# christhetree/mod_extraction

Hardware: AMD Instinct MI355X
Metric: 44.1 kHz audio-seconds/sec (train step), interwoven ph/fl/ch (higher is better)
Workload: dtype f32

## Files before the change

### mod_extraction_amd/csrc/wgrad_kvec_f16.hip

```cpp
#include "conv_common.h"
#include <stdlib.h>

typedef _Float16 half8 __attribute__((ext_vector_type(8)));
typedef _Float16 half4 __attribute__((ext_vector_type(4)));
typedef short short4v __attribute__((__vector_size__(4 * sizeof(short))));

#define WK_KS_MAX 6
#define WK_CH (WK_KS_MAX * 32)
#define WK_AP (WK_CH + 16)
#define WK_BR (WK_CH + 12)

#define WK_A_BYTES (2 * 64 * WK_AP * 2)
#define WK_B_ROWS ((WK_BR + 7) / 8 * 8)
#define WK_LDS_BYTES (WK_A_BYTES + 2 * WK_B_ROWS * 32)

struct WgradKvecArgs {
    const float *G;
    const unsigned char *amax;
    const float *scale;
    const _Float16 *xk_hi, *xk_lo;
    float *part;
    int B, H, Wv, rows_per_slab, n_slabs;
    int packed;
};

__device__ __forceinline__ floatx4 mfma_16x16x32(half8 a, half8 b, floatx4 c)
{
    return __builtin_amdgcn_mfma_f32_16x16x32_f16(a, b, c, 0, 0, 0);
}

__device__ __forceinline__ int wk_a_slot(int c8) { return c8 < 4 ? 8 * c8 : 8 * (c8 - 4) + 4; }
__device__ __forceinline__ half8 tr_frag16(const unsigned char *img, int lane_off, int r0)
{
    const unsigned char *ptr = img + lane_off + r0 * 32;
    const short4v v0 = __builtin_amdgcn_ds_read_tr16_b64_v4i16((short4v __attribute__((address_space(3))) *)ptr);
    const short4v v1 = __builtin_amdgcn_ds_read_tr16_b64_v4i16((short4v __attribute__((address_space(3))) *)(ptr + 16 * 32));
    typedef short short8v __attribute__((__vector_size__(8 * sizeof(short))));
    const short8v both = __builtin_shufflevector(v0, v1, 0, 1, 2, 3, 4, 5, 6, 7);
    return __builtin_bit_cast(half8, both);
}

__global__ __launch_bounds__(256, 2) void wgrad_kvec_f16_kernel(WgradKvecArgs a)
{
    extern __shared__ __attribute__((aligned(256))) unsigned char wk_smem[];
    _Float16 *const dzA = reinterpret_cast<_Float16 *>(wk_smem);
    _Float16 *const xB = reinterpret_cast<_Float16 *>(wk_smem + WK_A_BYTES);
    const int tid = threadIdx.x, lane = tid & 63, wave = __builtin_amdgcn_readfirstlane(tid >> 6);
    const int tap0 = wave * 3 + (wave >> 1);
    const int m16 = lane & 15, kg = lane >> 4;
    const int slab = blockIdx.x;
    const int Hp = a.H >> 1;
    const float S = a.scale[0];

    floatx4 acc[CV_KW];
#pragma unroll
    for (int i = 0; i < CV_KW; ++i) acc[i] = floatx4{0.f, 0.f, 0.f, 0.f};

    const int a_lane = (m16 * WK_AP + 8 * kg) * 2;
    const int b_lane = (4 * kg + (m16 >> 2)) * 32 + (m16 & 3) * 8;
    constexpr int A_SPLIT = 64 * WK_AP * 2, B_SPLIT = WK_B_ROWS * 32;
    const unsigned char *Ab = reinterpret_cast<const unsigned char *>(dzA);
    const unsigned char *Bb = reinterpret_cast<const unsigned char *>(xB);

    const int row_begin = slab * a.rows_per_slab;
    int row_end = row_begin + a.rows_per_slab;
    if (row_end > a.B * a.H) row_end = a.B * a.H;
    constexpr int NA = 64 * (WK_CH / 4) / 256, NB = (2 * WK_BR * 2 + 255) / 256;
    floatx4 ga[NA], vb[NB];
    unsigned ama[NA];
    auto issue_g = [&](int rid, int w0) {
        const int b = rid / a.H, h = rid - b * a.H;
        const int npos = (CV_PITCH - w0 >= WK_CH) ? WK_CH : (CV_PITCH - w0);
#pragma unroll
        for (int q = 0; q < NA; ++q) {
            const int i = tid + q * 256, co = i / (WK_CH / 4), c4 = i - co * (WK_CH / 4);
            ga[q] = floatx4{0.f, 0.f, 0.f, 0.f};
            ama[q] = 0x02020202u;
            if (c4 * 4 < npos) {
                const size_t off = (((size_t)b * 64 + co) * Hp + (h >> 1)) * CV_PITCH + w0 + c4 * 4;
                ga[q] = __builtin_nontemporal_load(reinterpret_cast<const floatx4 *>(a.G + off));
                ama[q] = __builtin_nontemporal_load(reinterpret_cast<const unsigned *>(a.amax + off));
            }
        }
    };
    auto issue_x = [&](int rid, int w0) {
        const int b = rid / a.H, h = rid - b * a.H;
        const int npos = (CV_PITCH - w0 >= WK_CH) ? WK_CH : (CV_PITCH - w0);
#pragma unroll
        for (int q = 0; q < NB; ++q) {
            const int i = tid + q * 256;
            const int split = i / (WK_BR * 2), k = i - split * (WK_BR * 2);
            const int pos = k >> 1, part = k & 1, w = w0 - 6 + pos;
            vb[q] = floatx4{0.f, 0.f, 0.f, 0.f};
            if (i < 2 * WK_BR * 2 && pos < npos + 12 && w >= 0 && w < CV_PITCH)
                vb[q] = *reinterpret_cast<const floatx4 *>((split ? a.xk_lo : a.xk_hi) +
                                                           (((size_t)b * a.H + h) * CV_PITCH + w) * 16 + part * 8);
        }
    };
    auto commit = [&](int rid, int w0) {
        const int h = rid % a.H;
        const unsigned want = (unsigned)(h & 1);
#pragma unroll
        for (int q = 0; q < NA; ++q) {
            const int i = tid + q * 256, co = i / (WK_CH / 4), c4 = i - co * (WK_CH / 4);
            const int wq = w0 + c4 * 4;
            half4 hi, lo;
            if (a.packed) {
                unsigned v[4];
#pragma unroll
                for (int e = 0; e < 4; ++e) v[e] = ((ama[q] >> (8 * e)) & 0xffu) == want ? __float_as_uint(ga[q][e]) : 0u;
                const unsigned h01 = __builtin_amdgcn_perm(v[1], v[0], 0x05040100u), h23 = __builtin_amdgcn_perm(v[3], v[2], 0x05040100u);
                const unsigned l01 = __builtin_amdgcn_perm(v[1], v[0], 0x07060302u), l23 = __builtin_amdgcn_perm(v[3], v[2], 0x07060302u);
                typedef unsigned uintx2 __attribute__((ext_vector_type(2)));
                hi = __builtin_bit_cast(half4, uintx2{h01, h23});
                lo = __builtin_bit_cast(half4, uintx2{l01, l23});
            } else {
#pragma unroll
            for (int e = 0; e < 4; ++e) {
                const bool keep = ((ama[q] >> (8 * e)) & 0xffu) == want && wq + e < a.Wv;
                const float v = keep ? ga[q][e] * S : 0.0f;
                const _Float16 hh = (_Float16)v;
                hi[e] = hh;
                lo[e] = (_Float16)(v - (float)hh);
            }
            }
            const int slot = (c4 >> 3) * 32 + wk_a_slot(c4 & 7);
            *reinterpret_cast<half4 *>(dzA + co * WK_AP + slot) = hi;
            *reinterpret_cast<half4 *>(dzA + 64 * WK_AP + co * WK_AP + slot) = lo;
        }
#pragma unroll
        for (int q = 0; q < NB; ++q) {
            const int i = tid + q * 256;
            if (i < 2 * WK_BR * 2) {
                const int split = i / (WK_BR * 2), k = i - split * (WK_BR * 2);
                *reinterpret_cast<floatx4 *>(xB + (size_t)split * (WK_B_ROWS * 16) + (k >> 1) * 16 + (k & 1) * 8) = vb[q];
            }
        }
    };

    int rid = row_begin, w0 = 0;
    if (rid < row_end) { issue_g(rid, w0); issue_x(rid, w0); }
    while (rid < row_end) {
        const int nks = (CV_PITCH - w0 >= WK_CH) ? WK_KS_MAX : (CV_PITCH - w0) / 32;
        int nrid, nw0 = w0;
        if (!(rid & 1)) nrid = rid + 1;
        else {
            nrid = rid - 1;
            nw0 = w0 + WK_CH;
            if (nw0 >= CV_PITCH) { nw0 = 0; nrid = rid + 1; }
        }
        __syncthreads();
        commit(rid, w0);
        if (nrid < row_end) {
            if (!(nrid & 1)) issue_g(nrid, nw0);
            issue_x(nrid, nw0);
        }
        __syncthreads();
        {
            {
#pragma unroll 1
            for (int ks = 0; ks < nks; ++ks) {
                half8 ah[5], al[5], bh[4], bl[4];
#pragma unroll
                for (int j = 0; j < 5; ++j) {
                    const int jt = j < 4 ? j : wave;
                    ah[j] = *reinterpret_cast<const half8 *>(Ab + a_lane + jt * (16 * WK_AP * 2) + ks * 64);
                    al[j] = *reinterpret_cast<const half8 *>(Ab + A_SPLIT + a_lane + jt * (16 * WK_AP * 2) + ks * 64);
                }
#pragma unroll
                for (int t = 0; t < 4; ++t) {
                    const int kw = t < 3 ? tap0 + t : 6;
                    bh[t] = tr_frag16(Bb, b_lane, ks * 32 + kw);
                    bl[t] = tr_frag16(Bb + B_SPLIT, b_lane, ks * 32 + kw);
                }
#pragma unroll
                for (int u = 0; u < 13; ++u) acc[u] = mfma_16x16x32(al[u < 12 ? (u & 3) : 4], bh[u < 12 ? (u >> 2) : 3], acc[u]);
#pragma unroll
                for (int u = 0; u < 13; ++u) acc[u] = mfma_16x16x32(ah[u < 12 ? (u & 3) : 4], bl[u < 12 ? (u >> 2) : 3], acc[u]);
#pragma unroll
                for (int u = 0; u < 13; ++u) acc[u] = mfma_16x16x32(ah[u < 12 ? (u & 3) : 4], bh[u < 12 ? (u >> 2) : 3], acc[u]);
            }
            }
        }
        rid = nrid;
        w0 = nw0;
    }
#pragma unroll
    for (int u = 0; u < CV_KW; ++u) {
        const int kw = u < 12 ? tap0 + (u >> 2) : 6, j = u < 12 ? (u & 3) : wave;
        float *dst = a.part + (((size_t)slab * CV_KW + kw) * 64 + j * 16) * 16;
#pragma unroll
        for (int r = 0; r < 4; ++r) dst[(4 * kg + r) * 16 + m16] = acc[u][r];
    }
}


__global__ __launch_bounds__(256) void wgrad_kvec_reduce_kernel(const float *__restrict__ part, int n_slabs,
                                                                const float *__restrict__ scale, float *__restrict__ dW)
{
    __shared__ double sh[16][17];
    const int total = CV_KW * 64 * 16;
    const int ol = threadIdx.x & 15, sl = threadIdx.x >> 4;
    const int j = blockIdx.x * 16 + ol;
    double s = 0.0;
    for (int i = sl; i < n_slabs; i += 16) s += (double)part[(size_t)i * total + j];
    sh[sl][ol] = s;
    __syncthreads();
    if (sl == 0) {
        double t = 0.0;
#pragma unroll
        for (int q = 0; q < 16; ++q) t += sh[q][ol];
        const int k = j & 15, co = (j >> 4) & 63, kw = j >> 10;
        if (k < 2 * CV_KH) {
            const int kh = k >> 1, ci = k & 1;
            dW[(((size_t)co * 2 + ci) * CV_KH + kh) * CV_KW + kw] = (float)(t * (double)scale[1]);
        }
    }
}

__global__ void wk_pow2_scale_kernel(const unsigned *__restrict__ amax_bits, float *__restrict__ scale)
{
    const float m = __uint_as_float(*amax_bits);
    int e = 0;
    if (m > 0.0f && m < 3.0e38f) {
        frexpf(m, &e);
        e = 10 - e;
        e = e > 100 ? 100 : (e < -100 ? -100 : e);
    }
    scale[0] = ldexpf(1.0f, e);
    scale[1] = ldexpf(1.0f, -e);
}

MX_EXPORT int mx_conv_block1_wgrad_f16(const float *G, const uint8_t *amax, const uint32_t *amax_bits, const void *xk_hi,
                                       const void *xk_lo, int64_t B, int64_t H, int64_t Wv, int64_t rows_per_slab,
                                       float *scale, float *part, float *dW, void *stream)
{
    if (!G || !amax || !amax_bits || !xk_hi || !xk_lo || !scale || !part || !dW || B <= 0 || rows_per_slab <= 0)
        return MX_ERR_ARG;
    if (H < 2 || (H & 1) || Wv <= 0 || Wv > CV_PITCH) return MX_ERR_UNSUPPORTED;
    rows_per_slab += rows_per_slab & 1;
    const int64_t n_slabs = (B * H + rows_per_slab - 1) / rows_per_slab;
    if (n_slabs > 1000000) return MX_ERR_UNSUPPORTED;
    hipStream_t st = (hipStream_t)stream;
    hipLaunchKernelGGL(wk_pow2_scale_kernel, dim3(1), dim3(1), 0, st, amax_bits, scale);
    WgradKvecArgs a{G, amax, scale, (const _Float16 *)xk_hi, (const _Float16 *)xk_lo, part, (int)B, (int)H, (int)Wv,
                    (int)rows_per_slab, (int)n_slabs, 0};
    static MxLdsLatch latch = {};
    if (mx_set_dyn_lds(latch, (const void *)wgrad_kvec_f16_kernel, WK_LDS_BYTES) != MX_OK) return MX_ERR_LAUNCH;
    hipLaunchKernelGGL(wgrad_kvec_f16_kernel, dim3((unsigned)n_slabs), dim3(256), WK_LDS_BYTES, st, a);
    const int total = CV_KW * 64 * 16;
    hipLaunchKernelGGL(wgrad_kvec_reduce_kernel, dim3(total / 16), dim3(256), 0, st, part, (int)n_slabs, scale, dW);
    return mx_launch_status();
}

MX_EXPORT int mx_conv_block1_wgrad_pair_f16(const void *Gp, const uint8_t *amax, const float *scale, const void *xk_hi,
                                            const void *xk_lo, int64_t B, int64_t H, int64_t Wv, int64_t rows_per_slab,
                                            float *part, float *dW, void *stream)
{
    if (!Gp || !amax || !scale || !xk_hi || !xk_lo || !part || !dW || B <= 0 || rows_per_slab <= 0) return MX_ERR_ARG;
    if (H < 2 || (H & 1) || Wv <= 0 || Wv > CV_PITCH) return MX_ERR_UNSUPPORTED;
    rows_per_slab += rows_per_slab & 1;
    const int64_t n_slabs = (B * H + rows_per_slab - 1) / rows_per_slab;
    if (n_slabs > 1000000) return MX_ERR_UNSUPPORTED;
    hipStream_t st = (hipStream_t)stream;
    WgradKvecArgs a{(const float *)Gp, amax, scale, (const _Float16 *)xk_hi, (const _Float16 *)xk_lo, part, (int)B, (int)H, (int)Wv,
                    (int)rows_per_slab, (int)n_slabs, 1};
    static MxLdsLatch latch = {};
    if (mx_set_dyn_lds(latch, (const void *)wgrad_kvec_f16_kernel, WK_LDS_BYTES) != MX_OK) return MX_ERR_LAUNCH;
    hipLaunchKernelGGL(wgrad_kvec_f16_kernel, dim3((unsigned)n_slabs), dim3(256), WK_LDS_BYTES, st, a);
    const int total = CV_KW * 64 * 16;
    hipLaunchKernelGGL(wgrad_kvec_reduce_kernel, dim3(total / 16), dim3(256), 0, st, part, (int)n_slabs, scale, dW);
    return mx_launch_status();
}
```

Baseline: 7730.

## Use 2:4 sparse SMFMAC for maxpool-masked wgrad, processing row pairs together

The weight-gradient kernel exploits the fact that the maxpool-backward gradient is nonzero in only one row of each H pair. It packs the row pair into a 2:4 structured-sparse A operand with per-lane index bytes and calls smfmac 16x16x64 instead of dense mfma 16x16x32. That halves the MFMA work and lets G/amax be loaded once per pair. The width chunk shrinks from 6 to 4 k-steps, and the LDS layout is reworked to hold interleaved x rows plus a sparsity index buffer. This adds extra index-packing ALU work and more complex transposed LDS reads.

```diff
diff --git a/mod_extraction_amd/csrc/wgrad_kvec_f16.hip b/mod_extraction_amd/csrc/wgrad_kvec_f16.hip
--- a/mod_extraction_amd/csrc/wgrad_kvec_f16.hip
+++ b/mod_extraction_amd/csrc/wgrad_kvec_f16.hip
@@ -1,18 +1,21 @@
 #include "conv_common.h"
 #include <stdlib.h>
 
+typedef _Float16 half16 __attribute__((ext_vector_type(16)));
 typedef _Float16 half8 __attribute__((ext_vector_type(8)));
 typedef _Float16 half4 __attribute__((ext_vector_type(4)));
 typedef short short4v __attribute__((__vector_size__(4 * sizeof(short))));
-
-#define WK_KS_MAX 6
+typedef unsigned uintx2 __attribute__((ext_vector_type(2)));
+
+#define WK_KS_MAX 4
 #define WK_CH (WK_KS_MAX * 32)
 #define WK_AP (WK_CH + 16)
 #define WK_BR (WK_CH + 12)
 
 #define WK_A_BYTES (2 * 64 * WK_AP * 2)
-#define WK_B_ROWS ((WK_BR + 7) / 8 * 8)
-#define WK_LDS_BYTES (WK_A_BYTES + 2 * WK_B_ROWS * 32)
+#define WK_B_SPLIT (WK_BR * 64)
+#define WK_I_BYTES (WK_KS_MAX * 512)
+#define WK_LDS_BYTES (WK_A_BYTES + 2 * WK_B_SPLIT + WK_I_BYTES)
 
 struct WgradKvecArgs {
     const float *G;
@@ -24,27 +27,32 @@
     int packed;
 };
 
-__device__ __forceinline__ floatx4 mfma_16x16x32(half8 a, half8 b, floatx4 c)
-{
-    return __builtin_amdgcn_mfma_f32_16x16x32_f16(a, b, c, 0, 0, 0);
-}
-
-__device__ __forceinline__ int wk_a_slot(int c8) { return c8 < 4 ? 8 * c8 : 8 * (c8 - 4) + 4; }
-__device__ __forceinline__ half8 tr_frag16(const unsigned char *img, int lane_off, int r0)
-{
-    const unsigned char *ptr = img + lane_off + r0 * 32;
-    const short4v v0 = __builtin_amdgcn_ds_read_tr16_b64_v4i16((short4v __attribute__((address_space(3))) *)ptr);
-    const short4v v1 = __builtin_amdgcn_ds_read_tr16_b64_v4i16((short4v __attribute__((address_space(3))) *)(ptr + 16 * 32));
+__device__ __forceinline__ floatx4 smfmac_16x16x64(half8 a, half16 b, floatx4 c, int idx)
+{
+    return __builtin_amdgcn_smfmac_f32_16x16x64_f16(a, b, c, idx, 0, 0);
+}
+
+__device__ __forceinline__ half16 tr_frag64(const unsigned char *img, int off_e, int off_o, int r0)
+{
+    typedef short4v __attribute__((address_space(3))) *lds_p;
+    const short4v v0 = __builtin_amdgcn_ds_read_tr16_b64_v4i16((lds_p)(img + off_e + r0));
+    const short4v v1 = __builtin_amdgcn_ds_read_tr16_b64_v4i16((lds_p)(img + off_o + r0));
+    const short4v v2 = __builtin_amdgcn_ds_read_tr16_b64_v4i16((lds_p)(img + off_e + r0 + 1024));
+    const short4v v3 = __builtin_amdgcn_ds_read_tr16_b64_v4i16((lds_p)(img + off_o + r0 + 1024));
     typedef short short8v __attribute__((__vector_size__(8 * sizeof(short))));
-    const short8v both = __builtin_shufflevector(v0, v1, 0, 1, 2, 3, 4, 5, 6, 7);
-    return __builtin_bit_cast(half8, both);
-}
-
-__global__ __launch_bounds__(256, 2) void wgrad_kvec_f16_kernel(WgradKvecArgs a)
+    typedef short short16v __attribute__((__vector_size__(16 * sizeof(short))));
+    const short8v lo = __builtin_shufflevector(v0, v1, 0, 1, 2, 3, 4, 5, 6, 7);
+    const short8v hi = __builtin_shufflevector(v2, v3, 0, 1, 2, 3, 4, 5, 6, 7);
+    const short16v all = __builtin_shufflevector(lo, hi, 0, 1, 2, 3, 4, 5, 6, 7, 8, 9, 10, 11, 12, 13, 14, 15);
+    return __builtin_bit_cast(half16, all);
+}
+
+__global__ __launch_bounds__(256, 2) void wgrad_kvec_sp_f16_kernel(WgradKvecArgs a)
 {
     extern __shared__ __attribute__((aligned(256))) unsigned char wk_smem[];
     _Float16 *const dzA = reinterpret_cast<_Float16 *>(wk_smem);
-    _Float16 *const xB = reinterpret_cast<_Float16 *>(wk_smem + WK_A_BYTES);
+    unsigned char *const Bb = wk_smem + WK_A_BYTES;
+    unsigned char *const Ib = wk_smem + WK_A_BYTES + 2 * WK_B_SPLIT;
     const int tid = threadIdx.x, lane = tid & 63, wave = __builtin_amdgcn_readfirstlane(tid >> 6);
     const int tap0 = wave * 3 + (wave >> 1);
     const int m16 = lane & 15, kg = lane >> 4;
@@ -57,132 +65,135 @@
     for (int i = 0; i < CV_KW; ++i) acc[i] = floatx4{0.f, 0.f, 0.f, 0.f};
 
     const int a_lane = (m16 * WK_AP + 8 * kg) * 2;
-    const int b_lane = (4 * kg + (m16 >> 2)) * 32 + (m16 & 3) * 8;
-    constexpr int A_SPLIT = 64 * WK_AP * 2, B_SPLIT = WK_B_ROWS * 32;
+    const int b_row = (kg & 1) * 256 + (kg >> 1) * 512 + (m16 >> 2) * 32 + (m16 & 3) * 8;
+    const int b_off_e = b_row + (kg & 1) * 128, b_off_o = b_row + (1 - (kg & 1)) * 128;
+    const int i_lane = lane * 8;
+    constexpr int A_SPLIT = 64 * WK_AP * 2;
     const unsigned char *Ab = reinterpret_cast<const unsigned char *>(dzA);
-    const unsigned char *Bb = reinterpret_cast<const unsigned char *>(xB);
-
-    const int row_begin = slab * a.rows_per_slab;
-    int row_end = row_begin + a.rows_per_slab;
-    if (row_end > a.B * a.H) row_end = a.B * a.H;
-    constexpr int NA = 64 * (WK_CH / 4) / 256, NB = (2 * WK_BR * 2 + 255) / 256;
+
+    const int pair_begin = (slab * a.rows_per_slab) >> 1;
+    int pair_end = pair_begin + (a.rows_per_slab >> 1);
+    if (pair_end > a.B * Hp) pair_end = a.B * Hp;
+    constexpr int NA = 64 * (WK_CH / 4) / 256, NB = (4 * WK_BR * 2 + 255) / 256;
     floatx4 ga[NA], vb[NB];
     unsigned ama[NA];
-    auto issue_g = [&](int rid, int w0) {
-        const int b = rid / a.H, h = rid - b * a.H;
+    const int c4 = tid & (WK_CH / 4 - 1), co0 = tid / (WK_CH / 4);
+    const bool odd = c4 & 1;
+    auto issue = [&](int pr, int w0) {
+        const int b = pr / Hp, hp = pr - b * Hp;
         const int npos = (CV_PITCH - w0 >= WK_CH) ? WK_CH : (CV_PITCH - w0);
 #pragma unroll
         for (int q = 0; q < NA; ++q) {
-            const int i = tid + q * 256, co = i / (WK_CH / 4), c4 = i - co * (WK_CH / 4);
+            const int co = co0 + q * (256 / (WK_CH / 4));
             ga[q] = floatx4{0.f, 0.f, 0.f, 0.f};
-            ama[q] = 0x02020202u;
+            ama[q] = 0u;
             if (c4 * 4 < npos) {
-                const size_t off = (((size_t)b * 64 + co) * Hp + (h >> 1)) * CV_PITCH + w0 + c4 * 4;
+                const size_t off = (((size_t)b * 64 + co) * Hp + hp) * CV_PITCH + w0 + c4 * 4;
                 ga[q] = __builtin_nontemporal_load(reinterpret_cast<const floatx4 *>(a.G + off));
                 ama[q] = __builtin_nontemporal_load(reinterpret_cast<const unsigned *>(a.amax + off));
             }
         }
-    };
-    auto issue_x = [&](int rid, int w0) {
-        const int b = rid / a.H, h = rid - b * a.H;
-        const int npos = (CV_PITCH - w0 >= WK_CH) ? WK_CH : (CV_PITCH - w0);
 #pragma unroll
         for (int q = 0; q < NB; ++q) {
             const int i = tid + q * 256;
-            const int split = i / (WK_BR * 2), k = i - split * (WK_BR * 2);
+            const int sp = i / (WK_BR * 2), k = i - sp * (WK_BR * 2);
             const int pos = k >> 1, part = k & 1, w = w0 - 6 + pos;
             vb[q] = floatx4{0.f, 0.f, 0.f, 0.f};
-            if (i < 2 * WK_BR * 2 && pos < npos + 12 && w >= 0 && w < CV_PITCH)
-                vb[q] = *reinterpret_cast<const floatx4 *>((split ? a.xk_lo : a.xk_hi) +
-                                                           (((size_t)b * a.H + h) * CV_PITCH + w) * 16 + part * 8);
+            if (i < 4 * WK_BR * 2 && pos < npos + 12 && w >= 0 && w < CV_PITCH)
+                vb[q] = *reinterpret_cast<const floatx4 *>(((sp >> 1) ? a.xk_lo : a.xk_hi) +
+                                                           (((size_t)b * a.H + 2 * hp + (sp & 1)) * CV_PITCH + w) * 16 + part * 8);
         }
     };
-    auto commit = [&](int rid, int w0) {
-        const int h = rid % a.H;
-        const unsigned want = (unsigned)(h & 1);
+    auto commit = [&](int w0) {
 #pragma unroll
         for (int q = 0; q < NA; ++q) {
-            const int i = tid + q * 256, co = i / (WK_CH / 4), c4 = i - co * (WK_CH / 4);
+            const int co = co0 + q * (256 / (WK_CH / 4));
             const int wq = w0 + c4 * 4;
-            half4 hi, lo;
+            const unsigned am = ama[q];
+            unsigned h01, h23, l01, l23;
             if (a.packed) {
                 unsigned v[4];
 #pragma unroll
-                for (int e = 0; e < 4; ++e) v[e] = ((ama[q] >> (8 * e)) & 0xffu) == want ? __float_as_uint(ga[q][e]) : 0u;
-                const unsigned h01 = __builtin_amdgcn_perm(v[1], v[0], 0x05040100u), h23 = __builtin_amdgcn_perm(v[3], v[2], 0x05040100u);
-                const unsigned l01 = __builtin_amdgcn_perm(v[1], v[0], 0x07060302u), l23 = __builtin_amdgcn_perm(v[3], v[2], 0x07060302u);
-                typedef unsigned uintx2 __attribute__((ext_vector_type(2)));
-                hi = __builtin_bit_cast(half4, uintx2{h01, h23});
-                lo = __builtin_bit_cast(half4, uintx2{l01, l23});
+                for (int e = 0; e < 4; ++e) v[e] = __float_as_uint(ga[q][e]);
+                if (am & 0xfefefefeu) {
+#pragma unroll
+                    for (int e = 0; e < 4; ++e) v[e] = ((am >> (8 * e)) & 0xfeu) ? 0u : v[e];
+                }
+                h01 = __builtin_amdgcn_perm(v[1], v[0], 0x05040100u), h23 = __builtin_amdgcn_perm(v[3], v[2], 0x05040100u);
+                l01 = __builtin_amdgcn_perm(v[1], v[0], 0x07060302u), l23 = __builtin_amdgcn_perm(v[3], v[2], 0x07060302u);
             } else {
-#pragma unroll
-            for (int e = 0; e < 4; ++e) {
-                const bool keep = ((ama[q] >> (8 * e)) & 0xffu) == want && wq + e < a.Wv;
-                const float v = keep ? ga[q][e] * S : 0.0f;
-                const _Float16 hh = (_Float16)v;
-                hi[e] = hh;
-                lo[e] = (_Float16)(v - (float)hh);
-            }
-            }
-            const int slot = (c4 >> 3) * 32 + wk_a_slot(c4 & 7);
-            *reinterpret_cast<half4 *>(dzA + co * WK_AP + slot) = hi;
-            *reinterpret_cast<half4 *>(dzA + 64 * WK_AP + co * WK_AP + slot) = lo;
+                half4 hi, lo;
+#pragma unroll
+                for (int e = 0; e < 4; ++e) {
+                    const bool keep = !((am >> (8 * e)) & 0xfeu) && wq + e < a.Wv;
+                    const float v = keep ? ga[q][e] * S : 0.0f;
+                    const _Float16 hh = (_Float16)v;
+                    hi[e] = hh;
+                    lo[e] = (_Float16)(v - (float)hh);
+                }
+                const uintx2 hw = __builtin_bit_cast(uintx2, hi), lw = __builtin_bit_cast(uintx2, lo);
+                h01 = hw.x, h23 = hw.y, l01 = lw.x, l23 = lw.y;
+            }
+            const unsigned ab = am & 0x01010101u;
+            unsigned t = ab | (ab >> 6);
+            t = (t | (t >> 12)) & 0x55u;
+            unsigned ib = t | 0x88u;
+            if (odd) ib = ((ib >> 4) | (ib << 4)) & 0xffu;
+            const uintx2 hs = odd ? uintx2{h23, h01} : uintx2{h01, h23};
+            const uintx2 ls = odd ? uintx2{l23, l01} : uintx2{l01, l23};
+            *reinterpret_cast<uintx2 *>(dzA + co * WK_AP + c4 * 4) = hs;
+            *reinterpret_cast<uintx2 *>(dzA + 64 * WK_AP + co * WK_AP + c4 * 4) = ls;
+            Ib[(c4 >> 1) * 128 + (co & 15) * 8 + (co >> 4) * 2 + (c4 & 1)] = (unsigned char)ib;
         }
 #pragma unroll
         for (int q = 0; q < NB; ++q) {
             const int i = tid + q * 256;
-            if (i < 2 * WK_BR * 2) {
-                const int split = i / (WK_BR * 2), k = i - split * (WK_BR * 2);
-                *reinterpret_cast<floatx4 *>(xB + (size_t)split * (WK_B_ROWS * 16) + (k >> 1) * 16 + (k & 1) * 8) = vb[q];
+            if (i < 4 * WK_BR * 2) {
+                const int sp = i / (WK_BR * 2), k = i - sp * (WK_BR * 2);
+                *reinterpret_cast<floatx4 *>(Bb + (sp >> 1) * WK_B_SPLIT + (k >> 1) * 64 + (sp & 1) * 32 + (k & 1) * 16) = vb[q];
             }
         }
     };
 
-    int rid = row_begin, w0 = 0;
-    if (rid < row_end) { issue_g(rid, w0); issue_x(rid, w0); }
-    while (rid < row_end) {
+    int pr = pair_begin, w0 = 0;
+    if (pr < pair_end) issue(pr, w0);
+    while (pr < pair_end) {
         const int nks = (CV_PITCH - w0 >= WK_CH) ? WK_KS_MAX : (CV_PITCH - w0) / 32;
-        int nrid, nw0 = w0;
-        if (!(rid & 1)) nrid = rid + 1;
-        else {
-            nrid = rid - 1;
-            nw0 = w0 + WK_CH;
-            if (nw0 >= CV_PITCH) { nw0 = 0; nrid = rid + 1; }
-        }
+        int npr = pr, nw0 = w0 + WK_CH;
+        if (nw0 >= CV_PITCH) { nw0 = 0; npr = pr + 1; }
         __syncthreads();
-        commit(rid, w0);
-        if (nrid < row_end) {
-            if (!(nrid & 1)) issue_g(nrid, nw0);
-            issue_x(nrid, nw0);
-        }
+        commit(w0);
+        if (npr < pair_end) issue(npr, nw0);
         __syncthreads();
-        {
-            {
 #pragma unroll 1
-            for (int ks = 0; ks < nks; ++ks) {
-                half8 ah[5], al[5], bh[4], bl[4];
-#pragma unroll
-                for (int j = 0; j < 5; ++j) {
-                    const int jt = j < 4 ? j : wave;
-                    ah[j] = *reinterpret_cast<const half8 *>(Ab + a_lane + jt * (16 * WK_AP * 2) + ks * 64);
-                    al[j] = *reinterpret_cast<const half8 *>(Ab + A_SPLIT + a_lane + jt * (16 * WK_AP * 2) + ks * 64);
-                }
-#pragma unroll
-                for (int t = 0; t < 4; ++t) {
-                    const int kw = t < 3 ? tap0 + t : 6;
-                    bh[t] = tr_frag16(Bb, b_lane, ks * 32 + kw);
-                    bl[t] = tr_frag16(Bb + B_SPLIT, b_lane, ks * 32 + kw);
-                }
-#pragma unroll
-                for (int u = 0; u < 13; ++u) acc[u] = mfma_16x16x32(al[u < 12 ? (u & 3) : 4], bh[u < 12 ? (u >> 2) : 3], acc[u]);
-#pragma unroll
-                for (int u = 0; u < 13; ++u) acc[u] = mfma_16x16x32(ah[u < 12 ? (u & 3) : 4], bl[u < 12 ? (u >> 2) : 3], acc[u]);
-#pragma unroll
-                for (int u = 0; u < 13; ++u) acc[u] = mfma_16x16x32(ah[u < 12 ? (u & 3) : 4], bh[u < 12 ? (u >> 2) : 3], acc[u]);
-            }
-            }
-        }
-        rid = nrid;
+        for (int ks = 0; ks < nks; ++ks) {
+            half8 ah[5], al[5];
+            int ix[5];
+            const uintx2 iw = *reinterpret_cast<const uintx2 *>(Ib + i_lane + ks * 512);
+            ix[0] = (int)(iw.x & 0xffffu), ix[1] = (int)(iw.x >> 16), ix[2] = (int)(iw.y & 0xffffu), ix[3] = (int)(iw.y >> 16);
+            ix[4] = (int)*reinterpret_cast<const unsigned short *>(Ib + i_lane + ks * 512 + wave * 2);
+#pragma unroll
+            for (int j = 0; j < 5; ++j) {
+                const int jt = j < 4 ? j : wave;
+                ah[j] = *reinterpret_cast<const half8 *>(Ab + a_lane + jt * (16 * WK_AP * 2) + ks * 64);
+                al[j] = *reinterpret_cast<const half8 *>(Ab + A_SPLIT + a_lane + jt * (16 * WK_AP * 2) + ks * 64);
+            }
+            const half16 bh6 = tr_frag64(Bb, b_off_e, b_off_o, ks * 2048 + 6 * 64);
+            const half16 bl6 = tr_frag64(Bb + WK_B_SPLIT, b_off_e, b_off_o, ks * 2048 + 6 * 64);
+#pragma unroll
+            for (int t = 0; t < 3; ++t) {
+                const half16 bh = tr_frag64(Bb, b_off_e, b_off_o, ks * 2048 + (tap0 + t) * 64);
+                const half16 bl = tr_frag64(Bb + WK_B_SPLIT, b_off_e, b_off_o, ks * 2048 + (tap0 + t) * 64);
+#pragma unroll
+                for (int j = 0; j < 4; ++j) acc[4 * t + j] = smfmac_16x16x64(ah[j], bl, acc[4 * t + j], ix[j]);
+                acc[12] = smfmac_16x16x64(t == 1 ? al[4] : ah[4], t == 0 ? bl6 : bh6, acc[12], ix[4]);
+#pragma unroll
+                for (int j = 0; j < 4; ++j) acc[4 * t + j] = smfmac_16x16x64(al[j], bh, acc[4 * t + j], ix[j]);
+#pragma unroll
+                for (int j = 0; j < 4; ++j) acc[4 * t + j] = smfmac_16x16x64(ah[j], bh, acc[4 * t + j], ix[j]);
+            }
+        }
+        pr = npr;
         w0 = nw0;
     }
 #pragma unroll
@@ -246,8 +257,8 @@
     WgradKvecArgs a{G, amax, scale, (const _Float16 *)xk_hi, (const _Float16 *)xk_lo, part, (int)B, (int)H, (int)Wv,
                     (int)rows_per_slab, (int)n_slabs, 0};
     static MxLdsLatch latch = {};
-    if (mx_set_dyn_lds(latch, (const void *)wgrad_kvec_f16_kernel, WK_LDS_BYTES) != MX_OK) return MX_ERR_LAUNCH;
-    hipLaunchKernelGGL(wgrad_kvec_f16_kernel, dim3((unsigned)n_slabs), dim3(256), WK_LDS_BYTES, st, a);
+    if (mx_set_dyn_lds(latch, (const void *)wgrad_kvec_sp_f16_kernel, WK_LDS_BYTES) != MX_OK) return MX_ERR_LAUNCH;
+    hipLaunchKernelGGL(wgrad_kvec_sp_f16_kernel, dim3((unsigned)n_slabs), dim3(256), WK_LDS_BYTES, st, a);
     const int total = CV_KW * 64 * 16;
     hipLaunchKernelGGL(wgrad_kvec_reduce_kernel, dim3(total / 16), dim3(256), 0, st, part, (int)n_slabs, scale, dW);
     return mx_launch_status();
@@ -266,8 +277,8 @@
     WgradKvecArgs a{(const float *)Gp, amax, scale, (const _Float16 *)xk_hi, (const _Float16 *)xk_lo, part, (int)B, (int)H, (int)Wv,
                     (int)rows_per_slab, (int)n_slabs, 1};
     static MxLdsLatch latch = {};
-    if (mx_set_dyn_lds(latch, (const void *)wgrad_kvec_f16_kernel, WK_LDS_BYTES) != MX_OK) return MX_ERR_LAUNCH;
-    hipLaunchKernelGGL(wgrad_kvec_f16_kernel, dim3((unsigned)n_slabs), dim3(256), WK_LDS_BYTES, st, a);
+    if (mx_set_dyn_lds(latch, (const void *)wgrad_kvec_sp_f16_kernel, WK_LDS_BYTES) != MX_OK) return MX_ERR_LAUNCH;
+    hipLaunchKernelGGL(wgrad_kvec_sp_f16_kernel, dim3((unsigned)n_slabs), dim3(256), WK_LDS_BYTES, st, a);
     const int total = CV_KW * 64 * 16;
     hipLaunchKernelGGL(wgrad_kvec_reduce_kernel, dim3(total / 16), dim3(256), 0, st, part, (int)n_slabs, scale, dW);
     return mx_launch_status();
```

Result: no change. 7772 (median of 6 runs) (+0.5%).
